# eRGiBi/DRL-DroneNavigation

Hardware: AMD Instinct MI355X
Metric: env_steps_per_sec (higher is better)
Workload: dtype f64

## Files before the change

drl-dronenavigation_amd/csrc/dn_kernels.hip:

```cpp
#include "dn_internal.h"
#include "dn_action_sat.h"

#ifndef DN_TU
#define DN_TU 1
#endif

#include <float.h>
#include <type_traits>

#define DN_DEV __device__ __forceinline__

namespace {

template <typename R> struct K {
    static constexpr R M = R(0.027);
    static constexpr R IXX = R(1.4e-5), IYY = R(1.4e-5), IZZ = R(2.17e-5);
    static constexpr R G = R(9.8);
    static constexpr R DT = R(1.0 / 240.0);
    static constexpr R ARM = R(0.028);
    static constexpr R LIN_DAMP = R(0.04), ANG_DAMP = R(0.04);
    static constexpr R MAX_COORD_VEL = R(100.0);
    static constexpr R PI = R(3.14159265358979323846);
    static constexpr R COLL_R = R(0.06), COLL_H = R(0.025);
    static constexpr R INV_M = R(1.0 / 0.027);
// ... 666 lines not shown
}

template <typename R>
DN_DEV void reset_obs(const DnParams &p, const DnConsts<R> &c, R d_last, float o[DN_OBS_DIM])
{
#pragma unroll
    for (int k = 0; k < 12; ++k) o[k] = c.reset_obs32[k];
    o[12] = p.include_distance ? (float)(d_last * c.inv_max_target_dist) : 0.0f;
}

struct Thrust {
    float f[4];
    float zt;
};
template <typename R> struct Flight {
    R px, py, pz, qx, qy, qz, qw;
    R fwx, fwy, fwz;
    float roll_num32, roll_den32, pitch32, yaw32;
    float vx, vy, vz, wx, wy, wz;
    float vex, vey, vez, aex, aey, aez;
    float d_e, dprev_e;
    int idx_e, just_found_e, truncated;
};
constexpr int DN_NMAIL64 = 7;
template <typename R> struct Verdict {
    R d_obs;
    int coll1;
    int terminated;
};

struct PidCtx {
    float4 G0, G1, G2;
    double *st;
};
DN_DEV void euler_from_quat64(const double q[4], double rpy[3])
{
    const double sqx = q[0] * q[0], sqy = q[1] * q[1], sqz = q[2] * q[2], squ = q[3] * q[3];
    const double sarg = -2.0 * (q[0] * q[2] - q[3] * q[1]);
    if (sarg <= -0.99999) { rpy[0] = 0.0; rpy[1] = -0.5 * 3.14159265358979323846; rpy[2] = 2.0 * atan2(q[0], -q[1]); }
    else if (sarg >= 0.99999) { rpy[0] = 0.0; rpy[1] = 0.5 * 3.14159265358979323846; rpy[2] = 2.0 * atan2(-q[0], q[1]); }
    else {
        rpy[0] = atan2(2.0 * (q[1] * q[2] + q[3] * q[0]), squ - sqx - sqy + sqz);
        rpy[1] = asin(sarg);
        rpy[2] = atan2(2.0 * (q[0] * q[1] + q[3] * q[2]), squ + sqx - sqy - sqz);
    }
}
// ... 253 lines not shown
template <typename R>
DN_DEV AttCol<R> attitude_column_terms(const float4 G1, const QuatTerms<R> &t)
{
    const R qx = G1.x, qy = G1.y;
    AttCol<R> c;
    c.r02 = F(qx, t.zs, t.wys); c.r12 = F(qy, t.zs, -t.wxs); c.r22 = R(1.0) - F(qx, t.xs, t.yy);
    return c;
}
template <typename R>
DN_DEV AttCol<R> attitude_column(const float4 G1)
{
    const R qx = G1.x, qy = G1.y, qz = G1.z, qw = G1.w;
    return attitude_column_terms<R>(G1, quat_terms<R>(qx, qy, qz, qw));
}
template <typename R> DN_DEV QuatTerms<R> quat_terms_identity()
{
    QuatTerms<R> t;
    t.xs = t.ys = t.zs = t.wxs = t.wys = t.wzs = t.yy = t.zz = R(0.0);
    return t;
}
template <typename R> struct LinPre {
    R vkx, vky, kl;
};
template <typename R>
DN_DEV LinPre<R> physics_linear_pre(const float4 G2, const R damp = K<R>::LIN_DAMP)
{
    LinPre<R> l;
    const R vx = G2.x, vy = G2.y, vz = G2.z;
    l.kl = F(damp, (R)__builtin_amdgcn_sqrtf((float)F(vz, vz, F(vy, vy, vx * vx))), damp);
    l.vkx = vx * l.kl; l.vky = vy * l.kl;
    return l;
}
template <typename R>
DN_DEV Lin<R> physics_linear_post(const float4 G0, const float4 G2, const AttCol<R> col, const LinPre<R> &l, const R fz, const R dax, const R day,
                                  const R daz, const bool extra, const R inv_m = K<R>::INV_M)
{
    Lin<R> o;
    R px = G0.x, py = G0.y, pz = G0.z;
    R vx = G2.x, vy = G2.y, vz = G2.z;
    const R dt = K<R>::DT;
    const R r02 = col.r02, r12 = col.r12, r22 = col.r22;
    const R fm = fz * inv_m;
    R awx = F(r02, fm, -l.vkx), awy = F(r12, fm, -l.vky), awz = F(-vz, l.kl, F(r22, fm, -K<R>::G));
    if (extra) { awx += dax; awy += day; awz += daz; }
    vx = F(awx, dt, vx); vy = F(awy, dt, vy); vz = F(awz, dt, vz);
    const R mv = K<R>::MAX_COORD_VEL;
    if (__builtin_expect(fmax(fmax(fabs(vx), fabs(vy)), fabs(vz)) > mv, 0)) {
        vx = clipv(vx, -mv, mv); vy = clipv(vy, -mv, mv); vz = clipv(vz, -mv, mv);
    }
    o.px = F(dt, vx, px); o.py = F(dt, vy, py); o.pz = F(dt, vz, pz);
    o.vx = vx; o.vy = vy; o.vz = vz;
    return o;
}
template <typename R>
DN_DEV Lin<R> physics_linear_col(const float4 G0, const float4 G2, const AttCol<R> col, const R fz, const R dax, const R day, const R daz,
                                 const bool extra, const R damp = K<R>::LIN_DAMP, const R inv_m = K<R>::INV_M)
{
    return physics_linear_post<R>(G0, G2, col, physics_linear_pre<R>(G2, damp), fz, dax, day, daz, extra, inv_m);
}
template <typename R>
DN_DEV Lin<R> physics_linear(const float4 G0, const float4 G1, const float4 G2, const R fz, const R dax, const R day, const R daz,
                             const bool extra, const R damp = K<R>::LIN_DAMP, const R inv_m = K<R>::INV_M)
{
    return physics_linear_col<R>(G0, G2, attitude_column<R>(G1), fz, dax, day, daz, extra, damp, inv_m);
}
template <typename R> struct Ang {
    R qx, qy, qz, qw;
    R wx, wy, wz;
};
template <typename R> struct AngPre {
    R qx, qy, qz, qw, wx, wy, wz;
    R r00, r01, r02, r10, r11, r12, r20, r21, r22;
    R ka, Iwx, Iwy, Iwz, gx, gy, gz;
};
template <typename R>
DN_DEV AngPre<R> physics_angular_pre_terms(const float4 G1, const float4 G3, const QuatTerms<R> &t, const R damp = K<R>::ANG_DAMP,
                                           const R ixx = K<R>::IXX, const R iyy = K<R>::IYY, const R izz = K<R>::IZZ);
template <typename R>
// ... 558 lines not shown
            const R cpit = cos(pitch);
            fwx = cos(yaw) * cpit; fwy = sin(yaw) * cpit; fwz = sin(pitch);
            pitch32 = (float)pitch; yaw32 = (float)yaw;
        } else {
            if (EULER) {
            roll_num32 = (float)(R(2.0) * FM<R>::fma(qy, qz, qw * qx));
            roll_den32 = (float)FM<R>::fma(qw, qw, FM<R>::fma(qz, qz, -FM<R>::fma(qx, qx, qy * qy)));
            yaw32 = atan2_fast32((float)ys, (float)yc);
            pitch32 = atan2_fast32((float)sarg, __builtin_amdgcn_sqrtf((float)FM<R>::fma(yc, yc, ys * ys)));
            } else { roll_num32 = 0.0f; roll_den32 = 1.0f; yaw32 = pitch32 = 0.0f; }
            fwx = yc; fwy = ys; fwz = sarg;
        }
    }
    fl.roll_num32 = roll_num32; fl.roll_den32 = roll_den32; fl.pitch32 = pitch32; fl.yaw32 = yaw32;
    fl.fwx = fwx; fl.fwy = fwy; fl.fwz = fwz;
}

template <typename R> struct Observed {
    float o[DN_OBS_DIM];
    R r_normal;
    float r_found32;
};

template <typename R>
DN_DEV void observe_columns_lin(const DnParams &p, const DnConsts<R> &c, const Flight<R> &fl, float o[DN_OBS_DIM])
{
    o[0] = (float)(fl.px * c.inv_dim[0]);
    o[1] = (float)(fl.py * c.inv_dim[1]);
    o[2] = (float)(fl.pz * c.inv_dim[2]);
    const float third32 = (float)K<R>::THIRD;
    const float v6 = (float)((R)fl.vx * K<R>::THIRD), v7 = (float)((R)fl.vy * K<R>::THIRD), v8 = (float)((R)fl.vz * K<R>::THIRD);
    o[6] = __builtin_amdgcn_fmed3f(v6, -1.0f, 1.0f);
    o[7] = __builtin_amdgcn_fmed3f(v7, -1.0f, 1.0f);
    o[8] = __builtin_amdgcn_fmed3f(v8, -third32, third32);
    if (__builtin_expect(__ballot(__builtin_isunordered(v6, v7) || v8 != v8) != 0ull, 0)) {
        o[6] = v6 != v6 ? v6 : o[6]; o[7] = v7 != v7 ? v7 : o[7]; o[8] = v8 != v8 ? v8 : o[8];
    }
    o[12] = p.include_distance ? (float)((R)fl.d_e * c.inv_max_target_dist) : 0.0f;
}
template <typename R>
DN_DEV void observe_columns_att(const Flight<R> &fl, float o[DN_OBS_DIM])
{
    const float roll32 = atan2_fast32(fl.roll_num32, fl.roll_den32), pitch32 = fl.pitch32, yaw32 = fl.yaw32;
    const float inv_pi32 = (float)K<R>::INV_PI;
    o[3] = roll32 * inv_pi32;
    o[4] = pitch32 * inv_pi32;
    o[5] = yaw32 * inv_pi32;
    const float w2f = __builtin_fmaf(fl.wz, fl.wz, __builtin_fmaf(fl.wy, fl.wy, fl.wx * fl.wx));
    const float rw32 = w2f != 0.0f ? __builtin_amdgcn_rsqf(w2f) : 0.0f;
    o[9] = fl.wx * rw32; o[10] = fl.wy * rw32; o[11] = fl.wz * rw32;
    if (__builtin_expect(w2f < 1e-30f && (fl.wx != 0.0f || fl.wy != 0.0f || fl.wz != 0.0f), 0)) {
        const R w2 = FM<R>::fma((R)fl.wz, (R)fl.wz, FM<R>::fma((R)fl.wy, (R)fl.wy, (R)fl.wx * (R)fl.wx));
        const R rw = FM<R>::rsq_f32grade(w2);
        o[9] = (float)((R)fl.wx * rw); o[10] = (float)((R)fl.wy * rw); o[11] = (float)((R)fl.wz * rw);
    }
}
template <typename R>
DN_DEV void observe_columns(const DnParams &p, const DnConsts<R> &c, const Flight<R> &fl, float o[DN_OBS_DIM])
{
    observe_columns_lin<R>(p, c, fl, o);
    observe_columns_att<R>(fl, o);
}
template <typename R> struct RewardPre {
    R r0;
    R s_lin, s_ang;
    bool pen_lin, pen_ang, found_now, last_gate;
};
template <typename R> struct Smooth {
    R s;
    bool pen;
};
template <typename R>
DN_DEV Smooth<R> smooth_term(const float ex, const float ey, const float ez, const float4 P, const R lim2)
{
    const R lx = (R)ex - (R)P.x, ly = (R)ey - (R)P.y, lz = (R)ez - (R)P.z;
    const R a2 = FM<R>::fma(lz, lz, FM<R>::fma(ly, ly, lx * lx));
    Smooth<R> o;
    o.pen = a2 > lim2;
    o.s = R(0.0);
    if (o.pen) o.s = (R)__builtin_amdgcn_sqrtf((float)a2);
    return o;
}
template <typename R>
DN_DEV void reward_entry_core(const DnParams &p, const DnConsts<R> &c, const Flight<R> &fl, RewardPre<R> &q)
{
    q.found_now = (R)fl.d_e <= c.threshold;
    q.last_gate = fl.idx_e + 1 == p.num_waypoints;
    const R gain = fl.just_found_e ? R(0.0) : ((R)fl.dprev_e - (R)fl.d_e) * R(3000.0);
    q.r0 = FM<R>::fma(R(3.0), (R)__builtin_amdgcn_exp2f((float)(R(-2.0 * 1.4426950408889634) * (R)fl.d_e)), gain);
}
template <typename R>
DN_DEV RewardPre<R> reward_entry(const DnParams &p, const DnConsts<R> &c, const Flight<R> &fl, const float4 G4, const float4 G5)
{
    RewardPre<R> q;
    reward_entry_core<R>(p, c, fl, q);
    const Smooth<R> sl = smooth_term<R>(fl.vex, fl.vey, fl.vez, G4, R(0.7) * R(0.7));
    const Smooth<R> sa = smooth_term<R>(fl.aex, fl.aey, fl.aez, G5, R(0.3) * R(0.3));
    q.pen_lin = sl.pen; q.pen_ang = sa.pen;
    q.s_lin = sl.s; q.s_ang = sa.s;
    return q;
}
template <typename R>
DN_DEV int reward_orientation(const DnParams &p, const R *s_tab, const Flight<R> &fl, const bool found_now, const bool last_gate)
{
    const int idx_ori = (found_now && !last_gate) ? fl.idx_e + 1 : fl.idx_e;
    return orientation_reward<R>(fl.fwx, fl.fwy, fl.fwz, fl.px, fl.py, fl.pz, s_tab + idx_ori * DN_T_STRIDE);
}
template <typename R>
DN_DEV void reward_assemble(const RewardPre<R> &q, const int ori, R &r_normal, float &r_found32)
{
    float r32 = 0.0f;
    if (q.last_gate) r32 = r32 + 200.0f;
    else { r32 = r32 + 75.0f; r32 = r32 + (float)(ori * 5); }
    r_found32 = r32;
    R r = q.r0 + (R)(ori * 3);
    if (q.pen_lin) r = r - q.s_lin;
    if (q.pen_ang) r = r - q.s_ang;
    r_normal = r;
}
template <typename R>
DN_DEV void reward_pose(const DnParams &p, const R *s_tab, const Flight<R> &fl, const RewardPre<R> &q, R &r_normal, float &r_found32)
{
    reward_assemble<R>(q, reward_orientation<R>(p, s_tab, fl, q.found_now, q.last_gate), r_normal, r_found32);
}
template <typename R>
DN_DEV void reward_candidates(const DnParams &p, const DnConsts<R> &c, const R *s_tab, const Flight<R> &fl, const float4 G4,
                              const float4 G5, R &r_normal, float &r_found32)
{
    const RewardPre<R> q = reward_entry<R>(p, c, fl, G4, G5);
    reward_pose<R>(p, s_tab, fl, q, r_normal, r_found32);
}
template <typename R, bool NORM, bool NOISE, bool SENS = false, bool PRIV = false, bool GOAL = false>
DN_DEV Observed<R> observe_phase(const DnParams &p, const DnConsts<R> &c, const R *s_tab, const Flight<R> &fl,
                                 const float4 G4, const float4 G5, const unsigned long long gid, const unsigned long long step_count,
                                 Rms &rms, SensCtx *sx = nullptr, const PrivCtx *px = nullptr, const GoalCtx<R> *gx = nullptr)
{
    Observed<R> ob;
    observe_columns<R>(p, c, fl, ob.o);
    if constexpr (PRIV) priv_true_obs(*px, ob.o);
    reward_candidates<R>(p, c, s_tab, fl, G4, G5, ob.r_normal, ob.r_found32);
    if (NOISE && p.obs_noise_sigma > 0.0f) add_obs_noise(p, gid, step_count, 1u, ob.o);
    if constexpr (SENS) sens_deliver(*sx, step_count, ob.o);
    if constexpr (GOAL) goal_observe<R>(*gx, p, c, ob.o);
    if (NORM) normalize_obs(rms, ob.o);
// ... 64 lines not shown

struct __attribute__((packed, aligned(4))) ObsQuad { float x, y, z, w; };
DN_DEV void store_obs_direct(float *row, const float o[DN_OBS_DIM])
{
    *reinterpret_cast<ObsQuad *>(row) = ObsQuad{o[0], o[1], o[2], o[3]};
    *reinterpret_cast<ObsQuad *>(row + 4) = ObsQuad{o[4], o[5], o[6], o[7]};
    *reinterpret_cast<ObsQuad *>(row + 8) = ObsQuad{o[8], o[9], o[10], o[11]};
    row[12] = o[12];
}
DN_DEV float ret_lo(const float hi, const int lenword)
{
    const int eb = (__float_as_int(hi) >> 23) & 0xFF;
    return (float)(lenword >> 24) * __int_as_float((eb > 31 ? eb - 31 : 0) << 23);
}
DN_DEV int ret_lo_byte(const double ep_ret, const float hi)
{
    const int eb = (__float_as_int(hi) >> 23) & 0xFF;
    const bool ok = eb > 31 && eb < 255;
    const float inv = __int_as_float((ok ? 285 - eb : 127) << 23);
    const double q = __builtin_rint((ep_ret - (double)hi) * (double)inv);
    const int k = (int)fmin(fmax(q, -128.0), 127.0);
    return ok ? (k & 0xFF) : 0;
}
template <typename R, bool REW>
DN_DEV void report_scalars(const DnParams &p, const DnConsts<R> &c, const StepOut &out, const Flight<R> &fl, const Verdict<R> &v,
                           const R r_normal, const float r_found32, const unsigned li, const unsigned lane, const bool active,
                           float4 &G4, float4 &G5, StatAcc &acc, RewNorm &rn)
{
    const bool coll1 = v.coll1 != 0, terminated = v.terminated != 0, truncated = fl.truncated != 0;
    const bool found_now = !coll1 && (R)fl.d_e <= c.threshold;
    const bool is_done = found_now && fl.idx_e + 1 == p.num_waypoints;
    const int found = fl.idx_e + (found_now ? 1 : 0);
    const bool done = terminated || truncated;
    R reward;
    if (coll1) reward = R(-10.0);
    else if (found_now) reward = (R)(r_found32 / 25.0f);
    else reward = r_normal * K<R>::INV_25;
    if (REW) reward = (R)reward_wrappers(p, rn, (double)reward, done);
    const int lenword = __float_as_int(G5.w);
    const int eplen_e = lenword & 0xFFFFFF;
    R ep_ret = ((R)G4.w + (R)ret_lo(G4.w, lenword)) + reward;
    int ep_len = eplen_e + 1;
    float4 S4 = G4, S5 = G5;
    if (!terminated) {
        S4 = make_float4(fl.vex, fl.vey, fl.vez, 0.0f);
        S5 = make_float4(fl.aex, fl.aey, fl.aez, 0.0f);
    }
    const unsigned long long done_ballot = __ballot(done && active);
    if (done_ballot != 0ull) {
        const long long fix = fixed6((double)ep_ret);
        if (done) {
            if (active) {
                if (out.ep_return) out.ep_return[li] = (float)ep_ret;
// ... 603 lines not shown
    for (int k = 0; k < 8; ++k) x[k] = m.f64[k][lane];
    f.px = x[0]; f.py = x[1]; f.pz = x[2]; f.qx = x[3]; f.qy = x[4]; f.qz = x[5]; f.qw = x[6];
    v.d_obs = x[7];
    const float4 a = m.f32[0][lane], b = m.f32[1][lane], c = m.f32[2][lane], d = m.f32[3][lane];
    f.vx = a.x; f.vy = a.y; f.vz = a.z; f.wx = a.w; f.wy = b.x; f.wz = b.y; f.vex = b.z; f.vey = b.w;
    f.vez = c.x; f.aex = c.y; f.aey = c.z; f.aez = c.w; f.d_e = d.x; f.dprev_e = d.y;
    const int bits = __float_as_int(d.z), vb = __float_as_int(d.w);
    f.idx_e = bits & 0xFF; f.just_found_e = (bits >> 8) & 1; f.truncated = (bits >> 9) & 1;
    v.coll1 = vb & 1; v.terminated = (vb >> 1) & 1;
}
template <typename R> struct MailA {
    R f64[2][DN_BLOCK];
    float4 f32[4][DN_BLOCK];
};
template <typename R> DN_DEV void post_maila(MailA<R> &m, unsigned lane, const Flight<R> &f, const Verdict<R> &v, const Observed<R> &ob)
{
    m.f64[0][lane] = ob.r_normal; m.f64[1][lane] = v.d_obs;
    const int bits = f.idx_e | (f.truncated << 9) | (v.coll1 << 10) | (v.terminated << 11);
    m.f32[0][lane] = make_float4(ob.o[0], ob.o[1], ob.o[2], ob.o[3]);
    m.f32[1][lane] = make_float4(ob.o[4], ob.o[5], ob.o[6], ob.o[7]);
    m.f32[2][lane] = make_float4(ob.o[8], ob.o[9], ob.o[10], ob.o[11]);
    m.f32[3][lane] = make_float4(ob.o[12], ob.r_found32, f.d_e, __int_as_float(bits));
}
template <typename R> DN_DEV void take_maila(const MailA<R> &m, unsigned lane, Flight<R> &f, Verdict<R> &v, Observed<R> &ob)
{
    ob.r_normal = m.f64[0][lane]; v.d_obs = m.f64[1][lane];
    const float4 a = m.f32[0][lane], b = m.f32[1][lane], c = m.f32[2][lane], d = m.f32[3][lane];
    ob.o[0] = a.x; ob.o[1] = a.y; ob.o[2] = a.z; ob.o[3] = a.w; ob.o[4] = b.x; ob.o[5] = b.y; ob.o[6] = b.z; ob.o[7] = b.w;
    ob.o[8] = c.x; ob.o[9] = c.y; ob.o[10] = c.z; ob.o[11] = c.w; ob.o[12] = d.x;
    ob.r_found32 = d.y; f.d_e = d.z;
    const int bits = __float_as_int(d.w);
    f.idx_e = bits & 0xFF; f.truncated = (bits >> 9) & 1; v.coll1 = (bits >> 10) & 1; v.terminated = (bits >> 11) & 1;
    f.vex = f.vey = f.vez = f.aex = f.aey = f.aez = 0.0f;
}

template <bool XOPT> struct ThrustMailX { double v[9][DN_BLOCK]; };
template <> struct ThrustMailX<false> { double v[1][1]; };
DN_DEV void post_thrust_x(ThrustMailX<true> &m, unsigned lane, const ThrustX &t, const Extras &x)
{
#pragma unroll
    for (int j = 0; j < 4; ++j) { m.v[j][lane] = t.f[j]; m.v[5 + j][lane] = x.rpm[j]; }
    m.v[4][lane] = t.zt;
}
DN_DEV void take_thrust_x(const ThrustMailX<true> &m, unsigned lane, ThrustX &t, Extras &x)
{
#pragma unroll
    for (int j = 0; j < 4; ++j) { t.f[j] = m.v[j][lane]; x.rpm[j] = m.v[5 + j][lane]; }
    t.zt = m.v[4][lane];
}
DN_DEV void post_thrust_x(ThrustMailX<false> &, unsigned, const ThrustX &, const Extras &) {}
DN_DEV void take_thrust_x(const ThrustMailX<false> &, unsigned, ThrustX &, Extras &) {}
template <typename R, bool XOPT> struct ThrustMailP : ThrustMail<R> {};
template <typename R> struct ThrustMailP<R, true> { R v[1][1]; };
template <typename R> DN_DEV void post_thrust(ThrustMailP<R, true> &, unsigned, const Thrust &) {}
template <typename R> DN_DEV Resultant<R> take_thrust(const ThrustMailP<R, true> &, unsigned) { return Resultant<R>(); }

// ... 122 lines not shown
                const unsigned long long sc = sc0 + (unsigned long long)u;
                Flight<R> fl;
                Verdict<R> v;
                Observed<R> ob;
                take_maila<R>(maila[u & 1], lane, fl, v, ob);
                if (NORM) normalize_obs(rms, ob.o);
                const StepOut out = block_out(io0, tile_base, (long long)u * n, (long long)u * words);
                report_phase<R, NORM, NOISE, XOPT, 2>(p, c, s_tile, out, fl, v, ob, gid, sc, li, lane, rows, active, G4, G5, acc, rms, rn);
            }
            if (t <= k_steps) block_lds_barrier();
        }
        flush_stats(p, acc, sc0 + (unsigned long long)k_steps, lane);
        if (NORM && active) store_rms(p, i, rms);
        if (XOPT && p.norm_rew && active) store_rewnorm(p, i, rn);
        if (active) {
            reinterpret_cast<float *>(b.g4 + li)[3] = G4.w;
            reinterpret_cast<float *>(b.g5 + li)[3] = G5.w;
            }
    }
}

template <typename R> struct MailL {
    R f64[4][DN_BLOCK];
    float4 f32[2][DN_BLOCK];
    int flags[DN_BLOCK];
};
template <typename R> struct MailG {
    R col[3][DN_BLOCK];
    R fw[3][DN_BLOCK];
    float4 eul[DN_BLOCK];
    float4 w[DN_BLOCK];
    float4 we[DN_BLOCK];
};

#ifdef DN_MW_STAMP
__device__ long long g_mw_stamp[8][48][2];
#define MW_MARK(k) do { if (lane == 0 && blockIdx.x == DN_MW_STAMP && t >= 8 && t < 56) \
        g_mw_stamp[role][t - 8][k] = (long long)__builtin_readcyclecounter(); } while (0)
#else
#define MW_MARK(k) do { } while (0)
#endif
#define MW_BARRIER() do { MW_MARK(0); block_lds_barrier(); MW_MARK(1); } while (0)
#ifdef DN_ROLE_MARK
#define MW_ROLE_MARK(name) asm volatile("; DN_ROLE_LOOP " name)
#else
#define MW_ROLE_MARK(name) do { } while (0)
#endif
#ifdef DN_MW_STAMP
__device__ long long g_mw_edge[16][8];
#define MW_EDGE(k) do { if (lane == 0 && (blockIdx.x == DN_MW_STAMP || blockIdx.x == DN_MW_STAMP + 256)) { const int r_ = role + (blockIdx.x == DN_MW_STAMP ? 0 : 8); \
        g_mw_edge[r_][k] = (long long)__builtin_readcyclecounter(); \
        if ((k) == 0) { g_mw_edge[r_][4] = (long long)wall_clock64(); g_mw_edge[r_][6] = (long long)__builtin_amdgcn_s_getreg(63492); } \
        if ((k) == 3) g_mw_edge[r_][5] = (long long)wall_clock64(); } } while (0)
#else
#define MW_EDGE(k) do { } while (0)
// ... 37 lines not shown
    const DnConsts<R> &c = consts<R>(p);
    const long long n = p.n, words = (p.n + 63) / 64;
    const unsigned long long sc0 = p.st.stats[blockIdx.x].step_count;
    MW_EDGE(0);
    stage_table<R>(p, s_tab);
#ifndef DN_5W_PRIO
#define DN_5W_PRIO "22311"
#endif
    {
        constexpr char pr[6] = DN_5W_PRIO;
        switch (pr[role] - '0') {
        case 1: __builtin_amdgcn_s_setprio(1); break;
        case 2: __builtin_amdgcn_s_setprio(2); break;
        case 3: __builtin_amdgcn_s_setprio(3); break;
        default: break;
        }
    }
    if (role == 0) {
        float4 G0 = b.g0[li], G2 = b.g2[li], G3 = b.g3[li];
        AttCol<R> col = attitude_column<R>(b.g1[li]);
        block_lds_barrier(); MW_EDGE(1);
        const R wp0[3] = {s_tab[DN_T_WP], s_tab[DN_T_WP + 1], s_tab[DN_T_WP + 2]};
        bool done_prev = false;
#pragma clang loop unroll(disable)
        for (int t = 0; t <= k_steps; ++t) {
            MW_ROLE_MARK("L");
            if (t < k_steps) {
                if (t > 0) {
                    const MailG<R> &mp = mailg[(t - 1) & 1];
                    const R c0 = mp.col[0][lane], c1 = mp.col[1][lane], c2 = mp.col[2][lane];
                    col.r02 = done_prev ? R(0.0) : c0; col.r12 = done_prev ? R(0.0) : c1; col.r22 = done_prev ? R(1.0) : c2;
                }
                const GateRow<R> row_e = load_gate_row<R>(s_tab, unpack_meta(G3.w).idx);
                const R fz = tmail[t & 1].v[0][lane];
                const Lin<R> lin = physics_linear_col<R>(G0, G2, col, fz, R(0.0), R(0.0), R(0.0), false);
                Flight<R> fl;
                flight_entry<R>(fl, G0, G2, G3, p.max_steps);
                fl.px = lin.px; fl.py = lin.py; fl.pz = lin.pz;
                fl.vx = (float)lin.vx; fl.vy = (float)lin.vy; fl.vz = (float)lin.vz;
                fl.qx = fl.qy = fl.qz = R(0.0); fl.qw = R(1.0);
                fl.wx = fl.wy = fl.wz = 0.0f;
                RulesMid<R> m;
                const Verdict<R> v = rules_verdict<R>(p, c, s_tab, row_e, fl, G3, m);
                MailL<R> &ml = maill[t & 1];
                ml.f64[0][lane] = fl.px; ml.f64[1][lane] = fl.py; ml.f64[2][lane] = fl.pz; ml.f64[3][lane] = v.d_obs;
                ml.f32[0][lane] = make_float4(fl.vx, fl.vy, fl.vz, fl.d_e);
                ml.f32[1][lane] = make_float4(fl.vex, fl.vey, fl.vez, fl.dprev_e);
                ml.flags[lane] = fl.idx_e | (fl.just_found_e << 8) | (fl.truncated << 9) | (v.coll1 << 10) | (v.terminated << 11);
                float4 S0, S1, S2, S3;
                rules_commit<R>(c, wp0, fl, m, G0, G3, b.g6, li, active, S0, S1, S2, S3);
                G0 = S0; G2 = S2; G3.w = S3.w;
                done_prev = v.terminated != 0 || fl.truncated != 0;
            }
            MW_BARRIER();
        }
        MW_EDGE(2);
        if (active) {
            b.g0[li] = G0; b.g2[li] = G2;
            reinterpret_cast<float *>(b.g3 + li)[3] = G3.w;
        }
    } else if (role == 1) {
        float4 G1 = b.g1[li], G3 = b.g3[li];
        QuatTerms<R> qt = quat_terms<R>((R)G1.x, (R)G1.y, (R)G1.z, (R)G1.w);
        block_lds_barrier(); MW_EDGE(1);
#pragma clang loop unroll(disable)
        for (int t = 0; t <= k_steps; ++t) {
            MW_ROLE_MARK("A");
            if (t > 0) {
                const int fb = maill[(t - 1) & 1].flags[lane];
                const bool fin = (((fb >> 9) | (fb >> 11)) & 1) != 0;
                if (__ballot(fin) != 0ull) {
                    if (fin) { G1 = make_float4(0.0f, 0.0f, 0.0f, 1.0f); G3.x = G3.y = G3.z = 0.0f; qt = quat_terms_identity<R>(); }
                }
            }
            if (t < k_steps) {
                const R tx = tmail[t & 1].v[1][lane], ty = tmail[t & 1].v[2][lane], zt = tmail[t & 1].v[3][lane];
                const Ang<R> ang = physics_angular_post<R>(physics_angular_pre_terms<R>(G1, G3, qt), tx, ty, zt);
                Flight<R> fl;
                fl.qx = ang.qx; fl.qy = ang.qy; fl.qz = ang.qz; fl.qw = ang.qw;
                attitude_phase<R>(fl);
                MailG<R> &mg = mailg[t & 1];
                const float4 qn = make_float4((float)ang.qx, (float)ang.qy, (float)ang.qz, (float)ang.qw);
                const float4 wn = make_float4((float)ang.wx, (float)ang.wy, (float)ang.wz, 0.0f);
                qt = quat_terms<R>((R)qn.x, (R)qn.y, (R)qn.z, (R)qn.w);
                const AttCol<R> cn = attitude_column_terms<R>(qn, qt);
                mg.col[0][lane] = cn.r02; mg.col[1][lane] = cn.r12; mg.col[2][lane] = cn.r22;
                mg.fw[0][lane] = fl.fwx; mg.fw[1][lane] = fl.fwy; mg.fw[2][lane] = fl.fwz;
                mg.eul[lane] = make_float4(fl.roll_num32, fl.roll_den32, fl.pitch32, fl.yaw32);
                mg.w[lane] = wn;
                mg.we[lane] = make_float4(G3.x, G3.y, G3.z, 0.0f);
                G1 = qn; G3.x = wn.x; G3.y = wn.y; G3.z = wn.z;
            }
            MW_BARRIER();
        }
        MW_EDGE(2);
        if (active) {
            b.g1[li] = G1;
            float *g3 = reinterpret_cast<float *>(b.g3 + li);
            g3[0] = G3.x; g3[1] = G3.y; g3[2] = G3.z;
        }
    } else if (role == 2) {
        float4 P4 = b.g4[li], P5 = b.g5[li];
        Rms rms;
        const float4 *act = reinterpret_cast<const float4 *>(io0.actions) + tile_base;
        float4 A = make_float4(0.0f, 0.0f, 0.0f, 0.0f);
        if (THRUST_ON_Q) {
            A = act[li];
            const float4 A1 = (act + (long long)(k_steps > 1 ? 1 : 0) * n)[li];
            post_thrust<R>(tmail[0], lane, thrust_phase<NOISE>(p, gid, sc0, A));
            A = A1;
        }
        block_lds_barrier(); MW_EDGE(1);
#pragma clang loop unroll(disable)
        for (int t = 0; t <= k_steps; ++t) {
            MW_ROLE_MARK("Q");
            if (THRUST_ON_Q && t + 1 < k_steps) {
                const float4 A_next = (act + (long long)(t + 2 < k_steps ? t + 2 : t + 1) * n)[li];
                post_thrust<R>(tmail[(t + 1) & 1], lane, thrust_phase<NOISE>(p, gid, sc0 + (unsigned long long)(t + 1), A));
                A = A_next;
            }
            if (t > 0) {
                const int u = t - 1;
                const MailL<R> &ml = maill[u & 1];
                const MailG<R> &mg = mailg[u & 1];
                Flight<R> fl;
                Verdict<R> v;
                fl.px = ml.f64[0][lane]; fl.py = ml.f64[1][lane]; fl.pz = ml.f64[2][lane]; v.d_obs = ml.f64[3][lane];
                const float4 a0 = ml.f32[0][lane], a1 = ml.f32[1][lane];
                fl.vx = a0.x; fl.vy = a0.y; fl.vz = a0.z; fl.d_e = a0.w;
                fl.vex = a1.x; fl.vey = a1.y; fl.vez = a1.z; fl.dprev_e = a1.w;
                const int fb = ml.flags[lane];
                fl.idx_e = fb & 0xFF; fl.just_found_e = (fb >> 8) & 1; fl.truncated = (fb >> 9) & 1;
                v.coll1 = (fb >> 10) & 1; v.terminated = (fb >> 11) & 1;
                const float4 e = mg.eul[lane], wn = mg.w[lane], we = mg.we[lane];
                fl.qx = fl.qy = fl.qz = R(0.0); fl.qw = R(1.0);
                fl.fwx = mg.fw[0][lane]; fl.fwy = mg.fw[1][lane]; fl.fwz = mg.fw[2][lane];
                fl.roll_num32 = e.x; fl.roll_den32 = e.y; fl.pitch32 = e.z; fl.yaw32 = e.w;
                fl.wx = wn.x; fl.wy = wn.y; fl.wz = wn.z;
                fl.aex = we.x; fl.aey = we.y; fl.aez = we.z;
                const Observed<R> ob = observe_phase<R, false, NOISE>(p, c, s_tab, fl, P4, P5, gid, sc0 + (unsigned long long)u, rms);
                post_maila<R>(maila[u & 1], lane, fl, v, ob);
                {
                    const bool fin = v.terminated != 0 || fl.truncated != 0;
                    P4 = fin ? make_float4(0.0f, 0.0f, 0.0f, 0.0f) : make_float4(fl.vex, fl.vey, fl.vez, 0.0f);
                    P5 = fin ? make_float4(0.0f, 0.0f, 0.0f, 0.0f) : make_float4(fl.aex, fl.aey, fl.aez, 0.0f);
                }
            }
            MW_BARRIER();
        }
        MW_EDGE(2);
        if (active) {
            float *g4 = reinterpret_cast<float *>(b.g4 + li), *g5 = reinterpret_cast<float *>(b.g5 + li);
            g4[0] = P4.x; g4[1] = P4.y; g4[2] = P4.z; g5[0] = P5.x; g5[1] = P5.y; g5[2] = P5.z;
        }
    } else if (role == 4) {
        Rms rms;
        load_rms(p, i, rms);
        block_lds_barrier(); MW_EDGE(1);
#pragma clang loop unroll(disable)
        for (int t = 0; t <= k_steps + 1; ++t) {
            MW_ROLE_MARK("N");
            if (t > 1) {
                const int u = t - 2;
                Flight<R> fl;
                Verdict<R> v;
                Observed<R> ob;
                take_maila<R>(maila[u & 1], lane, fl, v, ob);
                normalize_obs(rms, ob.o);
                const StepOut out = block_out(io0, tile_base, (long long)u * n, (long long)u * words);
                report_obs<R, NORM, NOISE, 2>(p, c, nullptr, out, fl.truncated != 0, v, ob.o, gid, sc0 + (unsigned long long)u, li, lane, rows, active, rms);
            }
            if (t <= k_steps) MW_BARRIER();
        }
        MW_EDGE(2);
        if (active) store_rms(p, i, rms);
    } else {
// ... 5 lines not shown
        const float4 *act = reinterpret_cast<const float4 *>(io0.actions) + tile_base;
        float4 A = make_float4(0.0f, 0.0f, 0.0f, 0.0f);
        if (!THRUST_ON_Q) {
            A = act[li];
            const float4 A1 = (act + (long long)(k_steps > 1 ? 1 : 0) * n)[li];
            post_thrust<R>(tmail[0], lane, thrust_phase<NOISE>(p, gid, sc0, A));
            A = A1;
        }
        block_lds_barrier(); MW_EDGE(1);
#pragma clang loop unroll(disable)
        for (int t = 0; t <= k_steps + 1; ++t) {
            MW_ROLE_MARK("X");
            if (!THRUST_ON_Q && t + 1 < k_steps) {
                const float4 A_next = (act + (long long)(t + 2 < k_steps ? t + 2 : t + 1) * n)[li];
                post_thrust<R>(tmail[(t + 1) & 1], lane, thrust_phase<NOISE>(p, gid, sc0 + (unsigned long long)(t + 1), A));
                A = A_next;
            }
            if (t > 1) {
                const int u = t - 2;
                const unsigned long long sc = sc0 + (unsigned long long)u;
                Flight<R> fl;
                Verdict<R> v;
                Observed<R> ob;
                take_maila<R>(maila[u & 1], lane, fl, v, ob);
                const StepOut out = block_out(io0, tile_base, (long long)u * n, (long long)u * words);
                if (NW == 5) report_scalars<R, false>(p, c, out, fl, v, ob.r_normal, ob.r_found32, li, lane, active, G4, G5, acc, rn);
                else {
                    if (NORM) normalize_obs(rms, ob.o);
                    report_phase<R, NORM, NOISE, false, 2>(p, c, nullptr, out, fl, v, ob, gid, sc, li, lane, rows, active, G4, G5, acc, rms, rn);
                }
            }
            if (t <= k_steps) MW_BARRIER();
        }
        MW_EDGE(2);
        flush_stats(p, acc, sc0 + (unsigned long long)k_steps, lane);
        if (NORM && NW == 4 && active) store_rms_walk(p, tile_base, li, rms);
        if (active) {
            reinterpret_cast<float *>(b.g4 + li)[3] = G4.w;
            reinterpret_cast<float *>(b.g5 + li)[3] = G5.w;
        }
    }
    MW_EDGE(3);
}

template <typename R, bool NORM, bool NOISE>
__global__ __launch_bounds__(4 * DN_BLOCK, 2) void dn_step_many_4w_kernel(const DnParams p, const DnStepIO io0, const int k_steps)
{
    step_many_4w_body<R, NORM, NOISE, 4>(p, io0, k_steps);
}
template <typename R, bool NOISE>
#ifndef DN_5W_WAVES_PER_EU
#define DN_5W_WAVES_PER_EU 4
#endif
// ... 1206 lines not shown
```

Measured before the change: 25.56 billion.

## Keep velocity and smoothing state in wide precision across warp-role mailboxes

Velocity, previous-velocity, angular-velocity-error and distance fields passed between the linear, angular and observe roles now travel through LDS mailboxes as R (double) instead of packed float4, so the observe role skips f32/f64 conversions. The observe role computes the reward inline using a new wide FlightW struct and sends a found bit in the mailbox flags. The report role uses that bit instead of recomputing the threshold test, and calls report_scalars/report_obs directly. This trades extra LDS footprint and traffic (doubles instead of floats) for fewer conversion instructions, and adds a profiling script that counts conversion ops per role.

Measured after the change: 25.86 billion (median of 6 runs). 1.2% higher.

```diff
diff --git a/drl-dronenavigation_amd/csrc/dn_kernels.hip b/drl-dronenavigation_amd/csrc/dn_kernels.hip
--- a/drl-dronenavigation_amd/csrc/dn_kernels.hip
+++ b/drl-dronenavigation_amd/csrc/dn_kernels.hip
@@ -712,6 +712,19 @@
     float d_e, dprev_e;
     int idx_e, just_found_e, truncated;
 };
+template <typename R> struct FlightW {
+    R px, py, pz, qx, qy, qz, qw;
+    R fwx, fwy, fwz;
+    float roll_num32, roll_den32, pitch32, yaw32;
+    R vx, vy, vz;
+    float wx, wy, wz;
+    R vex, vey, vez, aex, aey, aez;
+    R d_e, dprev_e;
+    int idx_e, just_found_e, truncated;
+};
+template <typename R> struct Vec3R {
+    R x, y, z;
+};
 constexpr int DN_NMAIL64 = 7;
 template <typename R> struct Verdict {
     R d_obs;
@@ -1011,8 +1024,8 @@
 template <typename R> struct LinPre {
     R vkx, vky, kl;
 };
-template <typename R>
-DN_DEV LinPre<R> physics_linear_pre(const float4 G2, const R damp = K<R>::LIN_DAMP)
+template <typename R, typename V>
+DN_DEV LinPre<R> physics_linear_pre(const V G2, const R damp = K<R>::LIN_DAMP)
 {
     LinPre<R> l;
     const R vx = G2.x, vy = G2.y, vz = G2.z;
@@ -1020,8 +1033,8 @@
     l.vkx = vx * l.kl; l.vky = vy * l.kl;
     return l;
 }
-template <typename R>
-DN_DEV Lin<R> physics_linear_post(const float4 G0, const float4 G2, const AttCol<R> col, const LinPre<R> &l, const R fz, const R dax, const R day,
+template <typename R, typename V>
+DN_DEV Lin<R> physics_linear_post(const float4 G0, const V G2, const AttCol<R> col, const LinPre<R> &l, const R fz, const R dax, const R day,
                                   const R daz, const bool extra, const R inv_m = K<R>::INV_M)
 {
     Lin<R> o;
@@ -1041,8 +1054,8 @@
     o.vx = vx; o.vy = vy; o.vz = vz;
     return o;
 }
-template <typename R>
-DN_DEV Lin<R> physics_linear_col(const float4 G0, const float4 G2, const AttCol<R> col, const R fz, const R dax, const R day, const R daz,
+template <typename R, typename V>
+DN_DEV Lin<R> physics_linear_col(const float4 G0, const V G2, const AttCol<R> col, const R fz, const R dax, const R day, const R daz,
                                  const bool extra, const R damp = K<R>::LIN_DAMP, const R inv_m = K<R>::INV_M)
 {
     return physics_linear_post<R>(G0, G2, col, physics_linear_pre<R>(G2, damp), fz, dax, day, daz, extra, inv_m);
@@ -1647,8 +1660,8 @@
     float r_found32;
 };
 
-template <typename R>
-DN_DEV void observe_columns_lin(const DnParams &p, const DnConsts<R> &c, const Flight<R> &fl, float o[DN_OBS_DIM])
+template <typename R, typename FL>
+DN_DEV void observe_columns_lin(const DnParams &p, const DnConsts<R> &c, const FL &fl, float o[DN_OBS_DIM])
 {
     o[0] = (float)(fl.px * c.inv_dim[0]);
     o[1] = (float)(fl.py * c.inv_dim[1]);
@@ -1663,8 +1676,8 @@
     }
     o[12] = p.include_distance ? (float)((R)fl.d_e * c.inv_max_target_dist) : 0.0f;
 }
-template <typename R>
-DN_DEV void observe_columns_att(const Flight<R> &fl, float o[DN_OBS_DIM])
+template <typename R, typename FL>
+DN_DEV void observe_columns_att(const FL &fl, float o[DN_OBS_DIM])
 {
     const float roll32 = atan2_fast32(fl.roll_num32, fl.roll_den32), pitch32 = fl.pitch32, yaw32 = fl.yaw32;
     const float inv_pi32 = (float)K<R>::INV_PI;
@@ -1707,7 +1720,18 @@
     return o;
 }
 template <typename R>
-DN_DEV void reward_entry_core(const DnParams &p, const DnConsts<R> &c, const Flight<R> &fl, RewardPre<R> &q)
+DN_DEV Smooth<R> smooth_term(const R ex, const R ey, const R ez, const Vec3R<R> &P, const R lim2)
+{
+    const R lx = ex - P.x, ly = ey - P.y, lz = ez - P.z;
+    const R a2 = FM<R>::fma(lz, lz, FM<R>::fma(ly, ly, lx * lx));
+    Smooth<R> o;
+    o.pen = a2 > lim2;
+    o.s = R(0.0);
+    if (o.pen) o.s = (R)__builtin_amdgcn_sqrtf((float)a2);
+    return o;
+}
+template <typename R, typename FL>
+DN_DEV void reward_entry_core(const DnParams &p, const DnConsts<R> &c, const FL &fl, RewardPre<R> &q)
 {
     q.found_now = (R)fl.d_e <= c.threshold;
     q.last_gate = fl.idx_e + 1 == p.num_waypoints;
@@ -1726,7 +1750,18 @@
     return q;
 }
 template <typename R>
-DN_DEV int reward_orientation(const DnParams &p, const R *s_tab, const Flight<R> &fl, const bool found_now, const bool last_gate)
+DN_DEV RewardPre<R> reward_entry(const DnParams &p, const DnConsts<R> &c, const FlightW<R> &fl, const Vec3R<R> &P4, const Vec3R<R> &P5)
+{
+    RewardPre<R> q;
+    reward_entry_core<R>(p, c, fl, q);
+    const Smooth<R> sl = smooth_term<R>(fl.vex, fl.vey, fl.vez, P4, R(0.7) * R(0.7));
+    const Smooth<R> sa = smooth_term<R>(fl.aex, fl.aey, fl.aez, P5, R(0.3) * R(0.3));
+    q.pen_lin = sl.pen; q.pen_ang = sa.pen;
+    q.s_lin = sl.s; q.s_ang = sa.s;
+    return q;
+}
+template <typename R, typename FL>
+DN_DEV int reward_orientation(const DnParams &p, const R *s_tab, const FL &fl, const bool found_now, const bool last_gate)
 {
     const int idx_ori = (found_now && !last_gate) ? fl.idx_e + 1 : fl.idx_e;
     return orientation_reward<R>(fl.fwx, fl.fwy, fl.fwz, fl.px, fl.py, fl.pz, s_tab + idx_ori * DN_T_STRIDE);
@@ -1743,8 +1778,8 @@
     if (q.pen_ang) r = r - q.s_ang;
     r_normal = r;
 }
-template <typename R>
-DN_DEV void reward_pose(const DnParams &p, const R *s_tab, const Flight<R> &fl, const RewardPre<R> &q, R &r_normal, float &r_found32)
+template <typename R, typename FL>
+DN_DEV void reward_pose(const DnParams &p, const R *s_tab, const FL &fl, const RewardPre<R> &q, R &r_normal, float &r_found32)
 {
     reward_assemble<R>(q, reward_orientation<R>(p, s_tab, fl, q.found_now, q.last_gate), r_normal, r_found32);
 }
@@ -1855,13 +1890,13 @@
     const int k = (int)fmin(fmax(q, -128.0), 127.0);
     return ok ? (k & 0xFF) : 0;
 }
-template <typename R, bool REW>
+template <typename R, bool REW, bool FOUND_BIT = false>
 DN_DEV void report_scalars(const DnParams &p, const DnConsts<R> &c, const StepOut &out, const Flight<R> &fl, const Verdict<R> &v,
                            const R r_normal, const float r_found32, const unsigned li, const unsigned lane, const bool active,
-                           float4 &G4, float4 &G5, StatAcc &acc, RewNorm &rn)
+                           float4 &G4, float4 &G5, StatAcc &acc, RewNorm &rn, const bool found_mail = false)
 {
     const bool coll1 = v.coll1 != 0, terminated = v.terminated != 0, truncated = fl.truncated != 0;
-    const bool found_now = !coll1 && (R)fl.d_e <= c.threshold;
+    const bool found_now = !coll1 && (FOUND_BIT ? found_mail : (R)fl.d_e <= c.threshold);
     const bool is_done = found_now && fl.idx_e + 1 == p.num_waypoints;
     const int found = fl.idx_e + (found_now ? 1 : 0);
     const bool done = terminated || truncated;
@@ -2511,7 +2546,7 @@
     m.f32[2][lane] = make_float4(ob.o[8], ob.o[9], ob.o[10], ob.o[11]);
     m.f32[3][lane] = make_float4(ob.o[12], ob.r_found32, f.d_e, __int_as_float(bits));
 }
-template <typename R> DN_DEV void take_maila(const MailA<R> &m, unsigned lane, Flight<R> &f, Verdict<R> &v, Observed<R> &ob)
+template <typename R> DN_DEV void take_maila(const MailA<R> &m, unsigned lane, Flight<R> &f, Verdict<R> &v, Observed<R> &ob, int *flag_word = nullptr)
 {
     ob.r_normal = m.f64[0][lane]; v.d_obs = m.f64[1][lane];
     const float4 a = m.f32[0][lane], b = m.f32[1][lane], c = m.f32[2][lane], d = m.f32[3][lane];
@@ -2521,6 +2556,18 @@
     const int bits = __float_as_int(d.w);
     f.idx_e = bits & 0xFF; f.truncated = (bits >> 9) & 1; v.coll1 = (bits >> 10) & 1; v.terminated = (bits >> 11) & 1;
     f.vex = f.vey = f.vez = f.aex = f.aey = f.aez = 0.0f;
+    if (flag_word) *flag_word = bits;
+}
+constexpr int DN_MAILA_FOUND_SHIFT = 12;
+template <typename R> DN_DEV void post_maila_found(MailA<R> &m, unsigned lane, const FlightW<R> &f, const Verdict<R> &v, const Observed<R> &ob,
+                                                   const bool found)
+{
+    m.f64[0][lane] = ob.r_normal; m.f64[1][lane] = v.d_obs;
+    const int bits = f.idx_e | (f.truncated << 9) | (v.coll1 << 10) | (v.terminated << 11) | ((int)found << DN_MAILA_FOUND_SHIFT);
+    m.f32[0][lane] = make_float4(ob.o[0], ob.o[1], ob.o[2], ob.o[3]);
+    m.f32[1][lane] = make_float4(ob.o[4], ob.o[5], ob.o[6], ob.o[7]);
+    m.f32[2][lane] = make_float4(ob.o[8], ob.o[9], ob.o[10], ob.o[11]);
+    m.f32[3][lane] = make_float4(ob.o[12], ob.r_found32, 0.0f, __int_as_float(bits));
 }
 
 template <bool XOPT> struct ThrustMailX { double v[9][DN_BLOCK]; };
@@ -2689,7 +2736,7 @@
 
 template <typename R> struct MailL {
     R f64[4][DN_BLOCK];
-    float4 f32[2][DN_BLOCK];
+    R wide[8][DN_BLOCK];
     int flags[DN_BLOCK];
 };
 template <typename R> struct MailG {
@@ -2697,7 +2744,7 @@
     R fw[3][DN_BLOCK];
     float4 eul[DN_BLOCK];
     float4 w[DN_BLOCK];
-    float4 we[DN_BLOCK];
+    R we[3][DN_BLOCK];
 };
 
 #ifdef DN_MW_STAMP
@@ -2781,6 +2828,7 @@
         block_lds_barrier(); MW_EDGE(1);
         const R wp0[3] = {s_tab[DN_T_WP], s_tab[DN_T_WP + 1], s_tab[DN_T_WP + 2]};
         bool done_prev = false;
+        Vec3R<R> W2 = {(R)G2.x, (R)G2.y, (R)G2.z};
 #pragma clang loop unroll(disable)
         for (int t = 0; t <= k_steps; ++t) {
             MW_ROLE_MARK("L");
@@ -2792,24 +2840,30 @@
                 }
                 const GateRow<R> row_e = load_gate_row<R>(s_tab, unpack_meta(G3.w).idx);
                 const R fz = tmail[t & 1].v[0][lane];
-                const Lin<R> lin = physics_linear_col<R>(G0, G2, col, fz, R(0.0), R(0.0), R(0.0), false);
+                const Lin<R> lin = physics_linear_col<R>(G0, W2, col, fz, R(0.0), R(0.0), R(0.0), false);
                 Flight<R> fl;
                 flight_entry<R>(fl, G0, G2, G3, p.max_steps);
                 fl.px = lin.px; fl.py = lin.py; fl.pz = lin.pz;
                 fl.vx = (float)lin.vx; fl.vy = (float)lin.vy; fl.vz = (float)lin.vz;
+                const Vec3R<R> Wn = {(R)fl.vx, (R)fl.vy, (R)fl.vz};
                 fl.qx = fl.qy = fl.qz = R(0.0); fl.qw = R(1.0);
                 fl.wx = fl.wy = fl.wz = 0.0f;
                 RulesMid<R> m;
                 const Verdict<R> v = rules_verdict<R>(p, c, s_tab, row_e, fl, G3, m);
                 MailL<R> &ml = maill[t & 1];
                 ml.f64[0][lane] = fl.px; ml.f64[1][lane] = fl.py; ml.f64[2][lane] = fl.pz; ml.f64[3][lane] = v.d_obs;
-                ml.f32[0][lane] = make_float4(fl.vx, fl.vy, fl.vz, fl.d_e);
-                ml.f32[1][lane] = make_float4(fl.vex, fl.vey, fl.vez, fl.dprev_e);
+                ml.wide[0][lane] = Wn.x; ml.wide[1][lane] = Wn.y; ml.wide[2][lane] = Wn.z;
+                ml.wide[3][lane] = W2.x; ml.wide[4][lane] = W2.y; ml.wide[5][lane] = W2.z;
+                ml.wide[6][lane] = (R)fl.d_e; ml.wide[7][lane] = (R)fl.dprev_e;
                 ml.flags[lane] = fl.idx_e | (fl.just_found_e << 8) | (fl.truncated << 9) | (v.coll1 << 10) | (v.terminated << 11);
                 float4 S0, S1, S2, S3;
                 rules_commit<R>(c, wp0, fl, m, G0, G3, b.g6, li, active, S0, S1, S2, S3);
                 G0 = S0; G2 = S2; G3.w = S3.w;
                 done_prev = v.terminated != 0 || fl.truncated != 0;
+                W2 = Wn;
+                if (__ballot(done_prev) != 0ull) {
+                    if (done_prev) W2.x = W2.y = W2.z = R(0.0);
+                }
             }
             MW_BARRIER();
         }
@@ -2833,12 +2887,13 @@
                 }
             }
             if (t < k_steps) {
+                MailG<R> &mg = mailg[t & 1];
+                mg.we[0][lane] = (R)G3.x; mg.we[1][lane] = (R)G3.y; mg.we[2][lane] = (R)G3.z;
                 const R tx = tmail[t & 1].v[1][lane], ty = tmail[t & 1].v[2][lane], zt = tmail[t & 1].v[3][lane];
                 const Ang<R> ang = physics_angular_post<R>(physics_angular_pre_terms<R>(G1, G3, qt), tx, ty, zt);
                 Flight<R> fl;
                 fl.qx = ang.qx; fl.qy = ang.qy; fl.qz = ang.qz; fl.qw = ang.qw;
                 attitude_phase<R>(fl);
-                MailG<R> &mg = mailg[t & 1];
                 const float4 qn = make_float4((float)ang.qx, (float)ang.qy, (float)ang.qz, (float)ang.qw);
                 const float4 wn = make_float4((float)ang.wx, (float)ang.wy, (float)ang.wz, 0.0f);
                 qt = quat_terms<R>((R)qn.x, (R)qn.y, (R)qn.z, (R)qn.w);
@@ -2847,7 +2902,6 @@
                 mg.fw[0][lane] = fl.fwx; mg.fw[1][lane] = fl.fwy; mg.fw[2][lane] = fl.fwz;
                 mg.eul[lane] = make_float4(fl.roll_num32, fl.roll_den32, fl.pitch32, fl.yaw32);
                 mg.w[lane] = wn;
-                mg.we[lane] = make_float4(G3.x, G3.y, G3.z, 0.0f);
                 G1 = qn; G3.x = wn.x; G3.y = wn.y; G3.z = wn.z;
             }
             MW_BARRIER();
@@ -2859,8 +2913,11 @@
             g3[0] = G3.x; g3[1] = G3.y; g3[2] = G3.z;
         }
     } else if (role == 2) {
-        float4 P4 = b.g4[li], P5 = b.g5[li];
-        Rms rms;
+        Vec3R<R> P4, P5;
+        {
+            const float4 g4 = b.g4[li], g5 = b.g5[li];
+            P4.x = (R)g4.x; P4.y = (R)g4.y; P4.z = (R)g4.z; P5.x = (R)g5.x; P5.y = (R)g5.y; P5.z = (R)g5.z;
+        }
         const float4 *act = reinterpret_cast<const float4 *>(io0.actions) + tile_base;
         float4 A = make_float4(0.0f, 0.0f, 0.0f, 0.0f);
         if (THRUST_ON_Q) {
@@ -2882,27 +2939,32 @@
                 const int u = t - 1;
                 const MailL<R> &ml = maill[u & 1];
                 const MailG<R> &mg = mailg[u & 1];
-                Flight<R> fl;
+                FlightW<R> fl;
                 Verdict<R> v;
                 fl.px = ml.f64[0][lane]; fl.py = ml.f64[1][lane]; fl.pz = ml.f64[2][lane]; v.d_obs = ml.f64[3][lane];
-                const float4 a0 = ml.f32[0][lane], a1 = ml.f32[1][lane];
-                fl.vx = a0.x; fl.vy = a0.y; fl.vz = a0.z; fl.d_e = a0.w;
-                fl.vex = a1.x; fl.vey = a1.y; fl.vez = a1.z; fl.dprev_e = a1.w;
+                fl.vx = ml.wide[0][lane]; fl.vy = ml.wide[1][lane]; fl.vz = ml.wide[2][lane];
+                fl.vex = ml.wide[3][lane]; fl.vey = ml.wide[4][lane]; fl.vez = ml.wide[5][lane];
+                fl.d_e = ml.wide[6][lane]; fl.dprev_e = ml.wide[7][lane];
                 const int fb = ml.flags[lane];
                 fl.idx_e = fb & 0xFF; fl.just_found_e = (fb >> 8) & 1; fl.truncated = (fb >> 9) & 1;
                 v.coll1 = (fb >> 10) & 1; v.terminated = (fb >> 11) & 1;
-                const float4 e = mg.eul[lane], wn = mg.w[lane], we = mg.we[lane];
+                const float4 e = mg.eul[lane], wn = mg.w[lane];
                 fl.qx = fl.qy = fl.qz = R(0.0); fl.qw = R(1.0);
                 fl.fwx = mg.fw[0][lane]; fl.fwy = mg.fw[1][lane]; fl.fwz = mg.fw[2][lane];
                 fl.roll_num32 = e.x; fl.roll_den32 = e.y; fl.pitch32 = e.z; fl.yaw32 = e.w;
                 fl.wx = wn.x; fl.wy = wn.y; fl.wz = wn.z;
-                fl.aex = we.x; fl.aey = we.y; fl.aez = we.z;
-                const Observed<R> ob = observe_phase<R, false, NOISE>(p, c, s_tab, fl, P4, P5, gid, sc0 + (unsigned long long)u, rms);
-                post_maila<R>(maila[u & 1], lane, fl, v, ob);
+                fl.aex = mg.we[0][lane]; fl.aey = mg.we[1][lane]; fl.aez = mg.we[2][lane];
+                Observed<R> ob;
+                observe_columns_lin<R>(p, c, fl, ob.o);
+                observe_columns_att<R>(fl, ob.o);
+                const RewardPre<R> pre = reward_entry<R>(p, c, fl, P4, P5);
+                reward_pose<R>(p, s_tab, fl, pre, ob.r_normal, ob.r_found32);
+                if (NOISE && p.obs_noise_sigma > 0.0f) add_obs_noise(p, gid, sc0 + (unsigned long long)u, 1u, ob.o);
+                post_maila_found<R>(maila[u & 1], lane, fl, v, ob, pre.found_now);
                 {
                     const bool fin = v.terminated != 0 || fl.truncated != 0;
-                    P4 = fin ? make_float4(0.0f, 0.0f, 0.0f, 0.0f) : make_float4(fl.vex, fl.vey, fl.vez, 0.0f);
-                    P5 = fin ? make_float4(0.0f, 0.0f, 0.0f, 0.0f) : make_float4(fl.aex, fl.aey, fl.aez, 0.0f);
+                    P4.x = fin ? R(0.0) : fl.vex; P4.y = fin ? R(0.0) : fl.vey; P4.z = fin ? R(0.0) : fl.vez;
+                    P5.x = fin ? R(0.0) : fl.aex; P5.y = fin ? R(0.0) : fl.aey; P5.z = fin ? R(0.0) : fl.aez;
                 }
             }
             MW_BARRIER();
@@ -2910,7 +2972,7 @@
         MW_EDGE(2);
         if (active) {
             float *g4 = reinterpret_cast<float *>(b.g4 + li), *g5 = reinterpret_cast<float *>(b.g5 + li);
-            g4[0] = P4.x; g4[1] = P4.y; g4[2] = P4.z; g5[0] = P5.x; g5[1] = P5.y; g5[2] = P5.z;
+            g4[0] = (float)P4.x; g4[1] = (float)P4.y; g4[2] = (float)P4.z; g5[0] = (float)P5.x; g5[1] = (float)P5.y; g5[2] = (float)P5.z;
         }
     } else if (role == 4) {
         Rms rms;
@@ -2962,13 +3024,14 @@
                 Flight<R> fl;
                 Verdict<R> v;
                 Observed<R> ob;
-                take_maila<R>(maila[u & 1], lane, fl, v, ob);
+                int fb;
+                take_maila<R>(maila[u & 1], lane, fl, v, ob, &fb);
+                const bool found_mail = ((fb >> DN_MAILA_FOUND_SHIFT) & 1) != 0;
                 const StepOut out = block_out(io0, tile_base, (long long)u * n, (long long)u * words);
-                if (NW == 5) report_scalars<R, false>(p, c, out, fl, v, ob.r_normal, ob.r_found32, li, lane, active, G4, G5, acc, rn);
-                else {
-                    if (NORM) normalize_obs(rms, ob.o);
-                    report_phase<R, NORM, NOISE, false, 2>(p, c, nullptr, out, fl, v, ob, gid, sc, li, lane, rows, active, G4, G5, acc, rms, rn);
-                }
+                if (NW != 5 && NORM) normalize_obs(rms, ob.o);
+                report_scalars<R, false, true>(p, c, out, fl, v, ob.r_normal, ob.r_found32, li, lane, active, G4, G5, acc, rn, found_mail);
+                if (NW != 5)
+                    report_obs<R, NORM, NOISE, 2>(p, c, nullptr, out, fl.truncated != 0, v, ob.o, gid, sc, li, lane, rows, active, rms);
             }
             if (t <= k_steps) MW_BARRIER();
         }
diff --git a/profiles/role_cvt.py b/profiles/role_cvt.py
--- /dev/null
+++ b/profiles/role_cvt.py
@@ -0,0 +1,98 @@
+#!/usr/bin/env python3
+import os
+import re
+import subprocess
+import sys
+import tempfile
+from collections import Counter
+
+ROOT = os.path.dirname(os.path.dirname(os.path.abspath(__file__)))
+KERN = "_ZN12_GLOBAL__N_122dn_step_many_5w_kernelIdLb0EEEv8DnParams8DnStepIOi"
+FLAGS = ["--offload-arch=gfx950", "-O3", "-std=c++17", "-fPIC", "-ffp-contract=off", "-fhip-fp32-correctly-rounded-divide-sqrt",
+         "-fno-fast-math", "--cuda-device-only", "-S", "-DDN_ROLE_MARK", "-Rpass-analysis=kernel-resource-usage"]
+TRANS = ("v_rsq", "v_rcp", "v_sqrt", "v_exp", "v_log", "v_sin", "v_cos")
+
+
+def role_loops(path):
+    body, on = [], False
+    for l in open(path):
+        if l.startswith(KERN + ":"):
+            on = True
+            continue
+        if on:
+            if l.startswith(".Lfunc_end"):
+                break
+            body.append(l.rstrip("\n"))
+    labels, ins, marks = {}, [], {}
+    for l in body:
+        m = re.match(r"^(\.LBB\d+_\d+):", l)
+        if m:
+            labels[m.group(1)] = len(ins)
+            continue
+        t = l.strip()
+        m = re.match(r"; DN_ROLE_LOOP (\w)", t)
+        if m:
+            marks[m.group(1)] = len(ins)
+            continue
+        if l.startswith("\t") and t and not t.startswith((".", ";")):
+            ins.append(t)
+    loops = {}
+    for name in "LAQNX":
+        start = marks[name]
+        hdr = max(v for v in labels.values() if v <= start)
+        end = None
+        for i in range(start, len(ins)):
+            m = re.match(r"s_cbranch\w*\s+(\.LBB\d+_\d+)|s_branch\s+(\.LBB\d+_\d+)", ins[i])
+            if m:
+                tgt = labels.get(m.group(1) or m.group(2))
+                if tgt is not None and tgt <= start and tgt >= hdr - 400:
+                    end = i
+            if i > start and any(i == v for k, v in marks.items() if k != name):
+                break
+        loops[name] = ins[hdr:end + 1]
+    return loops
+
+
+def table(loops):
+    print(f"{'role':4} {'cvt up':>7} {'cvt down':>9} {'f64 arith':>10} {'other VALU':>11} {'VALU':>6}")
+    tot = Counter()
+    for name in "LAQNX":
+        c = Counter(x.split()[0] for x in loops[name])
+        valu = sum(v for k, v in c.items() if k.startswith("v_"))
+        up = sum(v for k, v in c.items() if k.startswith("v_cvt_f64_f32"))
+        down = sum(v for k, v in c.items() if k.startswith("v_cvt_f32_f64"))
+        f64 = sum(v for k, v in c.items() if k.startswith("v_") and "f64" in k and not k.startswith(("v_cvt", "v_cmp") + TRANS))
+        row = dict(up=up, down=down, f64=f64, other=valu - up - down - f64, valu=valu)
+        tot.update(row)
+        print(f"{name:4} {up:7d} {down:9d} {f64:10d} {row['other']:11d} {valu:6d}")
+    print(f"{'sum':4} {tot['up']:7d} {tot['down']:9d} {tot['f64']:10d} {tot['other']:11d} {tot['valu']:6d}")
+
+
+def resources(remarks):
+    keys = ("VGPRs:", "ScratchSize", "Occupancy", "SGPRs Spill", "VGPRs Spill", "LDS Size")
+    on = False
+    for l in remarks.splitlines():
+        if "Function Name:" in l:
+            on = KERN in l
+        elif on and "remark:" in l and any(k in l for k in keys):
+            print("   ", l.split("remark:")[1].replace("[-Rpass-analysis=kernel-resource-usage]", "").strip())
+
+
+def main(argv):
+    if "--asm" in argv:
+        i = argv.index("--asm")
+        table(role_loops(argv[i + 1]))
+        return
+    with tempfile.TemporaryDirectory() as t:
+        out = os.path.join(t, "mw.s")
+        r = subprocess.run(["hipcc"] + FLAGS + argv + [os.path.join(ROOT, "drl-dronenavigation_amd", "csrc", "dn_kernels_mw.hip"), "-o", out],
+                           stderr=subprocess.PIPE, text=True)
+        if r.returncode != 0:
+            sys.exit(r.stderr)
+        table(role_loops(out))
+        print("dn_step_many_5w_kernel<double, false>:")
+        resources(r.stderr)
+
+
+if __name__ == "__main__":
+    main(sys.argv[1:])
```
